# haan6/fm-for-online-recommendation

Measured on AMD Instinct MI355X. Metric: samples/sec online-FM (Criteo-39-field, k=16) FTRL-proximal, higher is better.
Workload: dtype f32

## Files before the change

fm-for-online-recommendation_amd/csrc/fmx_common.h:

```cpp
#pragma once
#include <hip/hip_runtime.h>
#include <hip/hip_ext.h>

#include <cstdarg>
#include <cstdio>
#include <cstdlib>
#include <cstring>
#include <atomic>
#include <mutex>

#include "fmx.h"

#pragma clang fp contract(off)

namespace fmxd {
extern thread_local char g_err[512];
int fail(int code, const char *fmt, ...);
int check_launch(const char *what);

struct Tune {
  int wpb_fwd = 4, wpb_upd = 2;
  int sort_e = 0;
  int inline_fixup = 1;
  int upd_order = 1;
  int online_persistent = 1;
  int afm_online_persistent = 1;
  int afm_pair_online_persistent = 1;
  int sort_ahead = 16;
  int mlp_chain = 1;
  int sort_chunked = 1;
};
Tune &tune();

constexpr int UPD_ORDER_MAX = 128;

constexpr int FMX_COMM_SLOTS = 4;
struct Comm {
  int rank = 0, world = 1, n_blocks = 1;
  bool force = false;
  int block_count[FMX_COMM_MAX_WORLD] = {0}, block_first[FMX_COMM_MAX_WORLD] = {0};
  void *main = nullptr, *pf = nullptr;
  hipStream_t pf_stream = nullptr;
  hipEvent_t fork = nullptr, ready[FMX_COMM_SLOTS] = {nullptr}, free_[FMX_COMM_SLOTS] = {nullptr};
  bool used[FMX_COMM_SLOTS] = {false};
};
int comm_all_gather(Comm *c, int which, const void *send, void *recv, size_t count, hipStream_t st);
int comm_exchange_blocks(Comm *c, const float *send, float *recv, size_t per, hipStream_t st);

constexpr int MLP_BIG_MAX_L = 8;
struct MlpReduceArgs {
  const float *parts[MLP_BIG_MAX_L];
  int out_dim[MLP_BIG_MAX_L], in_dim[MLP_BIG_MAX_L], ldp[MLP_BIG_MAX_L];
  long long grad_off[MLP_BIG_MAX_L];
  float *grads;
  float *params;
  float lr;
  int rule;
  float *m, *v;
  float eps, c1, c2;
  int n_split[MLP_BIG_MAX_L], n_layers;
  const float *loss_b;
  float *loss_out;
  int B;
  float inv_b;
};
int mlp_section_deferred_reduce(const fmx_mlp_t *mlp, int32_t loss_kind, const float *bi, int32_t ld_bi, const float *base, const float *y, int32_t B,
                                float inv_b, void *workspace, float *logit_out, float *dz_out, float *gbi_out, int32_t ld_gbi, float *grads,
                                float lr_apply, float *loss_out, hipStream_t st, MlpReduceArgs *deferred, const char *who = "fmx_mlp_section",
                                float pair_margin = -1.f);
void mlp_launch_reduce(const MlpReduceArgs &a, hipStream_t st);
int mlp_opt_check(const fmx_mlp_t *mlp, int32_t B, const void *workspace, int64_t workspace_bytes, const float *grads, const fmx_mlp_opt_t *opt,
                  int64_t n_steps, const char *who);
int mlp_opt_state_check(const fmx_mlp_opt_t *opt, int64_t n_steps, const char *who);
int mlp_reduce_blocks_per_layer(const MlpReduceArgs &a, int threads);
}
using namespace fmxd;

namespace {

inline bool aligned16(const void *p) { return (reinterpret_cast<uintptr_t>(p) & 15u) == 0; }

constexpr uint32_t SENT = 0xFFFFFFFFu;
constexpr int WAVE = 64;
constexpr int LIST_MAX_G = 16;
constexpr int MAX_SORT_WIDTH = 32768;
constexpr int SORT_CHUNK = 1024;


__device__ __forceinline__ float4 operator+(float4 a, float4 b) { return {a.x + b.x, a.y + b.y, a.z + b.z, a.w + b.w}; }
__device__ __forceinline__ float4 operator-(float4 a, float4 b) { return {a.x - b.x, a.y - b.y, a.z - b.z, a.w - b.w}; }
__device__ __forceinline__ float4 operator*(float4 a, float4 b) { return {a.x * b.x, a.y * b.y, a.z * b.z, a.w * b.w}; }
__device__ __forceinline__ float4 operator*(float a, float4 b) { return {a * b.x, a * b.y, a * b.z, a * b.w}; }
__device__ __forceinline__ float4 splat(float a) { return {a, a, a, a}; }

__device__ __forceinline__ float4 shfl_xor4(float4 v, int m) {
  return {__shfl_xor(v.x, m), __shfl_xor(v.y, m), __shfl_xor(v.z, m), __shfl_xor(v.w, m)};
}
__device__ __forceinline__ float4 shfl_up4(float4 v, int d) {
  return {__shfl_up(v.x, d), __shfl_up(v.y, d), __shfl_up(v.z, d), __shfl_up(v.w, d)};
}
__device__ __forceinline__ float4 shfl4(float4 v, int src) {
  return {__shfl(v.x, src), __shfl(v.y, src), __shfl(v.z, src), __shfl(v.w, src)};
}

__device__ __forceinline__ float rcp_(float x) { return __builtin_amdgcn_rcpf(x); }
__device__ __forceinline__ float sqrt_(float x) { return __builtin_amdgcn_sqrtf(x); }

__device__ __forceinline__ float ftrl_w(float z, float n, const fmx_hyper_t &h) {
  const float denom = fmaf(h.beta + sqrt_(n), h.alpha, h.l2);
  const float w = -(z - copysignf(h.l1, z)) * rcp_(denom);
  return fabsf(z) <= h.l1 ? 0.f : w;
// ... 434 lines not shown
```

fm-for-online-recommendation_amd/csrc/fmx_host.h:

```cpp
#pragma once
#include <type_traits>

#include "fmx_common.h"

namespace fmxd {

struct Workspace {
  uint32_t *sorted;
  size_t sorted_stride;
  uint32_t *runs;
  int32_t *meta;
  int32_t *counter;
  float *parts;
  size_t bytes;
};

struct SortBatch {
  int n_pool = 1, first = 0, n_batches = 1;
  int64_t pool_stride = 0, sorted_stride = 0;
};

int check_table(const fmx_table_t *t);
int check_rule(const fmx_table_t *t, int rule);
int check_adam(const fmx_hyper_t *h, int rule, int64_t n_steps);
int check_sort_geometry(const fmx_table_t *t, int B);
int check_workspace(const fmx_table_t *t, int B, const void *workspace, int64_t workspace_bytes, const char *who);
int check_pair_args(const fmx_table_t *table, const fmx_hyper_t *hyper, const int32_t *idx, int64_t n_pairs, const char *count_name,
                    float margin, const char *who);
int check_list_args(const fmx_table_t *table, const fmx_hyper_t *hyper, const int32_t *idx, int32_t B_lists, int32_t G, int32_t *rows,
                    const char *who);
int named(int rc, const char *who);
int refuse_adaptive(int rule, const char *who);

int forward_impl(const fmx_table_t *table, const fmx_hyper_t *hyper, const int32_t *idx, const float *xv, const float *y,
                 int32_t B, int32_t loss_kind, float inv_b, const fmx_fwd_out_t *out, hipStream_t st);
int sort_impl(const fmx_table_t *table, const int32_t *idx, int32_t B, uint32_t *sorted, uint32_t *runs, int32_t *error,
              hipStream_t st, const SortBatch *mb = nullptr);
bool update_order(const fmx_table_t *table, bool may_fill, uint32_t *order_words);
int update_impl(const fmx_table_t *table, const fmx_hyper_t *hyper, int32_t rule, const Workspace &w,
                const uint32_t *sorted, const float *xv, const float *S, const float *dz_first, const float *dz_bi, const float *gbi,
                int32_t B, const float *loss_b, float inv_b, float *loss_out, hipStream_t st, int32_t *step_counter = nullptr,
                int32_t sample_ld = 0, int32_t *err_flag = nullptr, const MlpReduceArgs *rider = nullptr);
int update_occ_impl(const fmx_table_t *table, const fmx_hyper_t *hyper, int32_t rule, const Workspace &w, const float *xv,
                    const float *dz_first, const float *occ, int32_t ld_occ, int32_t B, const float *loss_b, float inv_b,
                    float *loss_out, hipStream_t st);
int afm_pair_online_buffers(int F, int k, int kp, int t, int attn_rule, bool *moments_in_lds);
int afm_pair_online_launch(const fmx_table_t *table, const fmx_hyper_t *hyper, int32_t rule, const fmx_afm_t *afm, const int32_t *idx,
                           const float *xv, int32_t N_pairs, float margin, float *attn_grad_out, const fmx_mlp_opt_t *opt,
                           float *logit_out, float *loss_out, int32_t *error, int nb, bool moments_in_lds, hipStream_t st);
int list_online_launch(const fmx_table_t *table, const fmx_hyper_t *hyper, int32_t rule, const int32_t *idx, const float *xv, int32_t N,
                       int32_t G, uint8_t *rank_out, float *logit_out, float *loss_out, int32_t *error, hipStream_t st);

}

namespace {

inline int lpr_of(int kp) {
  switch (kp) {
    case 4: return 1;
    case 8: return 2;
    case 16: return 4;
    case 32: return 8;
    case 64: return 16;
    default: return 0;
  }
}

template <class Fn>
decltype(auto) with_lpr(int kp, Fn &&f) {
  switch (lpr_of(kp)) {
    case 1: return f(std::integral_constant<int, 1>{});
    case 2: return f(std::integral_constant<int, 2>{});
    case 4: return f(std::integral_constant<int, 4>{});
    case 8: return f(std::integral_constant<int, 8>{});
    default: return f(std::integral_constant<int, 16>{});
  }
}

template <class Fn>
decltype(auto) with_kp(int kp, Fn &&f) {
  return with_lpr(kp, [&](auto LPR) { return f(std::integral_constant<int, 4 * LPR>{}); });
}

template <int... VS, class Fn>
bool with_one_of(int v, Fn &&f) {
  return ((v == VS && (f(std::integral_constant<int, VS>{}), true)) || ...);
}

template <bool MOMENTS_RULES, class Fn>
bool with_rule_impl(int rule, Fn &&f) {
  using Weights = std::integral_constant<int, FMX_LAYOUT_WEIGHTS>;
  using Moments = std::integral_constant<int, FMX_LAYOUT_MOMENTS>;
  switch (rule) {
    case FMX_RULE_SIGNADAM: f(Weights{}, std::integral_constant<int, FMX_RULE_SIGNADAM>{}); return true;
    case FMX_RULE_SGD: f(Weights{}, std::integral_constant<int, FMX_RULE_SGD>{}); return true;
    case FMX_RULE_FTRL: f(std::integral_constant<int, FMX_LAYOUT_FTRL>{}, std::integral_constant<int, FMX_RULE_FTRL>{}); return true;
    case FMX_RULE_ADAGRAD:
      if constexpr (MOMENTS_RULES) {
        f(Moments{}, std::integral_constant<int, FMX_RULE_ADAGRAD>{});
        return true;
      }
      return false;
    case FMX_RULE_ADAM:
      if constexpr (MOMENTS_RULES) {
        f(Moments{}, std::integral_constant<int, FMX_RULE_ADAM>{});
        return true;
      }
      return false;
    default: return false;
  }
}
template <class Fn>
bool with_rule(int rule, Fn &&f) { return with_rule_impl<true>(rule, f); }
template <class Fn>
bool with_rule_wf(int rule, Fn &&f) { return with_rule_impl<false>(rule, f); }

inline bool adaptive_rule(int rule) { return rule == FMX_RULE_ADAGRAD || rule == FMX_RULE_ADAM; }
inline const char *rule_name(int rule) { return rule == FMX_RULE_ADAM ? "FMX_RULE_ADAM" : "FMX_RULE_ADAGRAD"; }

inline bool mapped(const fmx_table_t *t) { return t->field_cols || t->field_base; }
inline int n_cols(const fmx_table_t *t) { return t->n_cols > 0 ? t->n_cols : t->n_fields; }
// ... 90 lines not shown
```

fm-for-online-recommendation_amd/csrc/fmx_kernels.hip:

```cpp

#include <cmath>

#include "fmx_host.h"

namespace fmxd {

thread_local char g_err[512] = "";

int fail(int code, const char *fmt, ...) {
  va_list ap;
  va_start(ap, fmt);
  vsnprintf(g_err, sizeof(g_err), fmt, ap);
  va_end(ap);
  return code;
}

int check_launch(const char *what) {
  hipError_t e = hipGetLastError();
  if (e != hipSuccess) return fail(FMX_ERR_LAUNCH, "%s: %s", what, hipGetErrorString(e));
  return FMX_OK;
}

}

// ... 444 lines not shown
int check_rule(const fmx_table_t *t, int rule) {
  if (rule == FMX_RULE_FTRL) {
    if (t->layout != FMX_LAYOUT_FTRL) return fail(FMX_ERR_ARG, "FMX_RULE_FTRL needs FMX_LAYOUT_FTRL");
  } else if (rule == FMX_RULE_SIGNADAM || rule == FMX_RULE_SGD) {
    if (t->layout != FMX_LAYOUT_WEIGHTS) return fail(FMX_ERR_ARG, "rule %d needs FMX_LAYOUT_WEIGHTS", rule);
  } else if (adaptive_rule(rule)) {
    if (t->layout != FMX_LAYOUT_MOMENTS) return fail(FMX_ERR_ARG, "%s needs FMX_LAYOUT_MOMENTS", rule_name(rule));
  } else {
    return fail(FMX_ERR_ARG, "unknown rule %d", rule);
  }
  return FMX_OK;
}

int check_adam(const fmx_hyper_t *h, int rule, int64_t n_steps) {
  if (rule != FMX_RULE_ADAM || !h) return FMX_OK;
  if (!(h->beta1 >= 0.f && h->beta1 < 1.f && h->beta2 >= 0.f && h->beta2 < 1.f))
    return fail(FMX_ERR_ARG, "FMX_RULE_ADAM: beta1 = %g and beta2 = %g must lie in [0, 1)", h->beta1, h->beta2);
  if (h->step < 0 || (int64_t)h->step + n_steps > INT32_MAX)
    return fail(FMX_ERR_ARG, "FMX_RULE_ADAM: step = %d must be >= 0 and step + steps of the call <= 2^31 - 1", h->step);
  return FMX_OK;
}

int check_sort_geometry(const fmx_table_t *t, int B) {
  if (B < 1) return fail(FMX_ERR_ARG, "B must be >= 1");
  const int Bp = fmx_sorted_width(B);
  if (Bp > MAX_SORT_WIDTH)
    return fail(FMX_ERR_UNSUPPORTED, "batch %d exceeds the LDS sort width %d", B, MAX_SORT_WIDTH);
  const int bbits = fmx_sorted_bbits(B);
  if ((uint64_t)(max_sort_rows(t) - 1) >= (uint64_t)(SENT >> bbits))
    return fail(FMX_ERR_UNSUPPORTED, "largest sort field (%lld rows) and batch %d do not fit a 32-bit (index, sample) composite: "
                "split the large fields (fmx_table_t.sort_offsets)", (long long)max_sort_rows(t), B);
  return FMX_OK;
}

int check_workspace(const fmx_table_t *t, int B, const void *workspace, int64_t workspace_bytes, const char *who) {
  if (!workspace) return fail(FMX_ERR_ARG, "%s: null workspace", who);
  if (!aligned16(workspace)) return fail(FMX_ERR_ALIGN, "%s: workspace must be 16-byte aligned", who);
  const int64_t need = (int64_t)carve(t, B, nullptr).bytes;
  if (workspace_bytes < need)
    return fail(FMX_ERR_SHAPE, "%s: workspace of %lld bytes, %lld needed for B = %d and %d sort fields (fmx_workspace_bytes)", who,
                (long long)workspace_bytes, (long long)need, B, n_sort_fields(t));
  return FMX_OK;
}

int named(int rc, const char *who) {
  if (rc != FMX_OK && !strstr(g_err, who)) {
    char msg[sizeof(g_err)];
    snprintf(msg, sizeof(msg), "%s", g_err);
    snprintf(g_err, sizeof(g_err), "%s: %s", who, msg);
  }
  return rc;
}

int check_pair_args(const fmx_table_t *table, const fmx_hyper_t *hyper, const int32_t *idx, int64_t n_pairs, const char *count_name,
                    float margin, const char *who) {
  if (!table) return fail(FMX_ERR_ARG, "%s: table is null", who);
  if (int rc = check_table(table)) return named(rc, who);
  if (!hyper) return fail(FMX_ERR_ARG, "%s: hyper is null", who);
  if (!idx) return fail(FMX_ERR_ARG, "%s: idx is null", who);
  if (n_pairs < 1) return fail(FMX_ERR_ARG, "%s: %s = %lld must be >= 1", who, count_name, (long long)n_pairs);
  if (!(margin >= 0.f) || !std::isfinite(margin)) return fail(FMX_ERR_ARG, "%s: margin = %g must be finite and >= 0", who, (double)margin);
  if (mapped(table))
    return fail(FMX_ERR_UNSUPPORTED, "%s: tables whose fields are pieces of index columns (field_cols / field_base) are not taken", who);
  return FMX_OK;
}

int check_list_args(const fmx_table_t *table, const fmx_hyper_t *hyper, const int32_t *idx, int32_t B_lists, int32_t G, int32_t *rows,
                    const char *who) {
  if (int rc = check_pair_args(table, hyper, idx, B_lists, "B_lists", 0.f, who)) return rc;
  if (G < 2) return fail(FMX_ERR_ARG, "%s: G = %d: a list is a positive and at least one negative (G >= 2)", who, G);
  if (G > LIST_MAX_G) return fail(FMX_ERR_UNSUPPORTED, "%s: G = %d: at most %d rows per list (one workgroup holds a list's waves)", who, G, LIST_MAX_G);
  if ((int64_t)B_lists * G > INT32_MAX) return fail(FMX_ERR_ARG, "%s: B_lists = %d, G = %d: B_lists * G rows exceed int32", who, B_lists, G);
  *rows = B_lists * G;
  return FMX_OK;
}

Tune &tune() {
  static Tune t = [] {
    Tune x;
    if (const char *e = getenv("FMX_WPB_FWD")) x.wpb_fwd = atoi(e);
    if (const char *e = getenv("FMX_WPB_UPD")) x.wpb_upd = atoi(e);
    if (const char *e = getenv("FMX_SORT_E")) x.sort_e = atoi(e);
    if (const char *e = getenv("FMX_SORT_AHEAD")) x.sort_ahead = atoi(e);
    if (const char *e = getenv("FMX_ONLINE_PERSISTENT")) x.online_persistent = atoi(e);
    if (const char *e = getenv("FMX_INLINE_FIXUP")) x.inline_fixup = atoi(e);
    if (const char *e = getenv("FMX_SORT_CHUNKED")) x.sort_chunked = atoi(e);
    if (const char *e = getenv("FMX_UPD_ORDER")) x.upd_order = atoi(e);
    if (const char *e = getenv("FMX_MLP_CHAIN")) x.mlp_chain = atoi(e);
    auto ok = [](int v) { return v == 1 || v == 2 || v == 4; };
    if (!ok(x.wpb_fwd)) x.wpb_fwd = 4;
    if (!ok(x.wpb_upd)) x.wpb_upd = 2;
    return x;
  }();
  return t;
}
}
namespace {

struct Side {
  hipStream_t stream = nullptr;
  hipStream_t main = nullptr;
  hipEvent_t fork = nullptr, sorted[2] = {nullptr, nullptr}, consumed[2] = {nullptr, nullptr};
  hipEvent_t user_fork = nullptr, user_join = nullptr;
};

Side *side_for_current_device() {
  static std::mutex mu;
  static Side sides[64];
  int dev = 0;
  if (hipGetDevice(&dev) != hipSuccess || dev < 0 || dev >= 64) return nullptr;
  std::lock_guard<std::mutex> lock(mu);
  Side &sd = sides[dev];
  if (!sd.stream) {
    int lo = 0, hi = 0;
    (void)hipDeviceGetStreamPriorityRange(&lo, &hi);
    if (hipStreamCreateWithPriority(&sd.stream, hipStreamNonBlocking, lo) != hipSuccess) return nullptr;
    if (hipStreamCreateWithPriority(&sd.main, hipStreamNonBlocking, hi) != hipSuccess) return nullptr;
    bool ok = hipEventCreateWithFlags(&sd.fork, hipEventDisableTiming) == hipSuccess &&
              hipEventCreateWithFlags(&sd.user_fork, hipEventDisableTiming) == hipSuccess &&
              hipEventCreateWithFlags(&sd.user_join, hipEventDisableTiming) == hipSuccess;
    for (int i = 0; i < 2 && ok; ++i) {
      ok = hipEventCreateWithFlags(&sd.sorted[i], hipEventDisableTiming) == hipSuccess &&
           hipEventCreateWithFlags(&sd.consumed[i], hipEventDisableTiming) == hipSuccess;
    }
    if (!ok) return nullptr;
  }
  return &sd;
}

struct UpdOrders {
  struct Entry {
    const int64_t *offs = nullptr;
    int F = 0;
    int64_t n_rows = 0, max_rows = 0;
    bool known = false;
    uint8_t order[2][UPD_ORDER_MAX];
  };
  static constexpr int N = 8;
  Entry e[N];
  int next = 0;
};

}
namespace fmxd {

bool update_order(const fmx_table_t *table, bool may_fill, uint32_t *order_words) {
  memset(order_words, 0, UPD_ORDER_MAX);
  const int mode = tune().upd_order, F = n_sort_fields(table);
  if ((mode != 1 && mode != 2) || F < 1 || F > UPD_ORDER_MAX) return false;
  static std::mutex mu;
  static UpdOrders per_device[64];
  int dev = 0;
  if (hipGetDevice(&dev) != hipSuccess || dev < 0 || dev >= 64) return false;
  const int64_t *offs = sort_offsets(table);
  std::lock_guard<std::mutex> lock(mu);
  UpdOrders &c = per_device[dev];
  UpdOrders::Entry *hit = nullptr;
  for (UpdOrders::Entry &x : c.e)
    if (x.offs == offs && x.F == F && x.n_rows == table->n_rows && x.max_rows == max_sort_rows(table)) hit = &x;
  if (!hit) {
    if (!may_fill) return false;
    hit = &c.e[c.next];
    c.next = (c.next + 1) % UpdOrders::N;
    hit->offs = offs;
    hit->F = F;
    hit->n_rows = table->n_rows;
    hit->max_rows = max_sort_rows(table);
    int64_t off[UPD_ORDER_MAX + 1], rows[UPD_ORDER_MAX];
    hipStreamCaptureMode cm = hipStreamCaptureModeRelaxed;
    const bool swapped = hipThreadExchangeStreamCaptureMode(&cm) == hipSuccess;
    hit->known = hipMemcpy(off, offs, sizeof(int64_t) * (size_t)(F + 1), hipMemcpyDeviceToHost) == hipSuccess;
    if (swapped) (void)hipThreadExchangeStreamCaptureMode(&cm);
    if (!hit->known) (void)hipGetLastError();
    for (int f = 0; f < F && hit->known; ++f) rows[f] = off[f + 1] - off[f];
    if (hit->known) hit->known = upd_order_of(rows, F, 1, hit->order[0]) == F && upd_order_of(rows, F, 2, hit->order[1]) == F;
  }
  if (!hit->known) return false;
  memcpy(order_words, hit->order[mode - 1], (size_t)F);
  return true;
}

}
namespace {

constexpr int OVERLAP_MIN_BATCH = 512;

template <int LPR, int NPASS, bool MAPPED = false, bool PAIR = false>
void launch_forward_np(const FwdArgs &a, int layout, hipStream_t st) {
  const int wpb = PAIR && tune().wpb_fwd < 2 ? 2 : tune().wpb_fwd;
  const dim3 grid((a.B + wpb - 1) / wpb), block(64 * wpb);
  if (layout == FMX_LAYOUT_FTRL) hipLaunchKernelGGL((k_fm_forward<LPR, FMX_LAYOUT_FTRL, NPASS, MAPPED, PAIR>), grid, block, 0, st, a);
  else hipLaunchKernelGGL((k_fm_forward<LPR, FMX_LAYOUT_WEIGHTS, NPASS, MAPPED, PAIR>), grid, block, 0, st, a);
}

template <int LPR, bool PAIR = false>
void launch_forward(const FwdArgs &a, int layout, hipStream_t st) {
  const int slots = WAVE / LPR;
  const int np = (a.F + slots - 1) / slots;
  if constexpr (!PAIR) {
    if (a.fcols || a.fbase) {
      launch_forward_np<LPR, 0, true>(a, layout, st);
      return;
    }
  }
  if (!with_one_of<1, 2, 3, 4>(np, [&](auto NP) { launch_forward_np<LPR, NP, false, PAIR>(a, layout, st); }))
    launch_forward_np<LPR, 0, false, PAIR>(a, layout, st);
}

template <int LPR, bool Q = false>
void launch_forward_list(const FwdArgs &a, int layout, hipStream_t st) {
  const int G = a.list_g, wpb = G * (4 / G > 1 ? 4 / G : 1);
  const dim3 grid((a.B + wpb - 1) / wpb), block(64 * wpb);
  const int slots = WAVE / LPR, np = (a.F + slots - 1) / slots;
  auto launch = [&](auto NP) {
    if constexpr (Q) {
      if (layout == FMX_LAYOUT_FTRL) hipLaunchKernelGGL((k_fm_forward_listq<LPR, FMX_LAYOUT_FTRL, NP>), grid, block, 0, st, a);
      else hipLaunchKernelGGL((k_fm_forward_listq<LPR, FMX_LAYOUT_WEIGHTS, NP>), grid, block, 0, st, a);
    } else {
      if (layout == FMX_LAYOUT_FTRL) hipLaunchKernelGGL((k_fm_forward_list<LPR, FMX_LAYOUT_FTRL, NP>), grid, block, 0, st, a);
      else hipLaunchKernelGGL((k_fm_forward_list<LPR, FMX_LAYOUT_WEIGHTS, NP>), grid, block, 0, st, a);
    }
  };
  if (!with_one_of<1, 2, 3, 4>(np, launch)) launch(std::integral_constant<int, 0>{});
}

template <int E>
void launch_sort(SortArgs a, hipStream_t st) {
  const int threads = a.Bp / E;
  uint32_t lds = (uint32_t)(a.Bp * sizeof(uint32_t));
  if (a.Bp <= RADIX_SMALL_WIDTH && threads >= 64) {
    a.small_bits = RADIX_SMALL_BITS;
    const uint32_t need = (uint32_t)radix_small_lds_bytes(a.Bp, threads);
    if (need > lds) lds = need;
  }
  const int grid = a.n_batches >= 8 ? 8 * a.F * ((a.n_batches + 7) / 8) : a.F * a.n_batches;
  hipLaunchKernelGGL((k_sort_occ<E>), dim3(grid), dim3(threads), lds, st, a);
}

int prepare_sort(int B) {
  if ((size_t)fmx_sorted_width(B) * 4 <= 64 * 1024) return FMX_OK;
  static std::mutex mu;
  static bool raised = false;
  std::lock_guard<std::mutex> lock(mu);
  if (!raised) {
    hipError_t e = hipFuncSetAttribute(reinterpret_cast<const void *>(k_sort_occ<8>), hipFuncAttributeMaxDynamicSharedMemorySize, MAX_SORT_WIDTH * 4);
    if (e == hipSuccess) e = hipFuncSetAttribute(reinterpret_cast<const void *>(k_sort_occ<16>), hipFuncAttributeMaxDynamicSharedMemorySize, MAX_SORT_WIDTH * 4);
    if (e == hipSuccess) e = hipFuncSetAttribute(reinterpret_cast<const void *>(k_sort_occ<32>), hipFuncAttributeMaxDynamicSharedMemorySize, MAX_SORT_WIDTH * 4);
    if (e != hipSuccess) return fail(FMX_ERR_LAUNCH, "hipFuncSetAttribute: %s", hipGetErrorString(e));
    raised = true;
  }
  return FMX_OK;
}

int prepare_merge(int Bp) {
  if ((size_t)(Bp + Bp / 32) * 4 <= 64 * 1024) return FMX_OK;
  static std::mutex mu;
  static bool raised = false;
  std::lock_guard<std::mutex> lock(mu);
  if (!raised) {
    hipError_t e = hipFuncSetAttribute(reinterpret_cast<const void *>(k_sort_merge), hipFuncAttributeMaxDynamicSharedMemorySize,
                                       (MAX_SORT_WIDTH + MAX_SORT_WIDTH / 32) * 4);
    if (e != hipSuccess) return fail(FMX_ERR_LAUNCH, "hipFuncSetAttribute: %s", hipGetErrorString(e));
    raised = true;
  }
  return FMX_OK;
}

}

int fmxd::sort_impl(const fmx_table_t *table, const int32_t *idx, int32_t B, uint32_t *sorted, uint32_t *runs, int32_t *error,
                    hipStream_t st, const SortBatch *mb) {
  SortArgs a;
  a.n_pool = mb ? mb->n_pool : 1;
  a.pool_first = mb ? mb->first : 0;
  a.n_batches = mb ? mb->n_batches : 1;
  a.pool_stride = mb ? mb->pool_stride : 0;
  a.sorted_stride = mb ? mb->sorted_stride : 0;
  a.idx = idx;
  a.foff = table->field_offsets;
  a.soff = sort_offsets(table);
  a.cols = sort_cols(table);
  a.sorted = sorted;
  a.error = error;
  a.B = B;
  a.F = n_sort_fields(table);
  a.Fi = n_cols(table);
  a.small_bits = 0;
  a.fcols = table->field_cols;
  a.fbase = table->field_base;
  a.Bp = fmx_sorted_width(B);
  a.bbits = fmx_sorted_bbits(B);
  if (a.Bp >= (tune().sort_chunked > 1 ? 2 * SORT_CHUNK : SORT_CHUNKED_MIN_WIDTH) && tune().sort_chunked && runs &&
      (a.n_batches <= 2 || tune().sort_chunked > 1)) {
    if (int rc = prepare_merge(a.Bp)) return rc;
    ChunkArgs c;
    c.s = a;
    c.runs = runs;
    c.runs_stride = (int64_t)align_up((size_t)a.F * a.Bp * 4, 256) / 4;
    c.C = a.Bp / SORT_CHUNK;
    const int units1 = a.n_batches * c.C, grid1 = 8 * a.F * ((units1 + 7) / 8);
    hipLaunchKernelGGL(k_sort_chunk, dim3(grid1), dim3(SORT_CHUNK_THREADS), 0, st, c);
    const int units2 = a.n_batches * a.F, grid2 = 8 * c.C * ((units2 + 7) / 8);
    hipLaunchKernelGGL(k_sort_merge, dim3(grid2), dim3(SORT_CHUNK_THREADS), (uint32_t)((a.Bp + a.Bp / 32) * sizeof(uint32_t)), st, c);
    return check_launch("k_sort_chunk / k_sort_merge");
  }
  if (int rc = prepare_sort(B)) return rc;
  int E = a.Bp <= 64 ? 1 : a.Bp <= 128 ? 2 : a.Bp <= 4096 ? 4 : a.Bp <= 8192 ? 8 : a.Bp <= 16384 ? 16 : 32;
  const int want = tune().sort_e;
  if (want > E && want <= 32 && (want & (want - 1)) == 0 && a.Bp / want >= 64) E = want;
  if (!with_one_of<1, 2, 4, 8, 16>(E, [&](auto E_) { launch_sort<E_>(a, st); })) launch_sort<32>(a, st);
  return check_launch("k_sort_occ");
}

namespace {

int sort_pool(const fmx_table_t *table, const int32_t *idx_pool, int n_pool, int B, int first_step, int n, const Workspace &w,
              uint32_t *sorted, int32_t *error, hipStream_t st) {
  SortBatch mb;
  mb.n_pool = n_pool;
  mb.first = first_step % n_pool;
  mb.n_batches = n;
  mb.pool_stride = (int64_t)B * (int64_t)n_cols(table);
  mb.sorted_stride = (int64_t)w.sorted_stride;
  return sort_impl(table, idx_pool, B, sorted, w.runs, error, st, &mb);
}

struct Detour {
  Side *sd;
  hipStream_t user, st;
  Detour(Side *side, hipStream_t stream) : sd(stream == nullptr ? side : nullptr), user(stream), st(stream) {
    if (!sd) return;
    (void)hipEventRecord(sd->user_fork, user);
    st = sd->main;
    (void)hipStreamWaitEvent(st, sd->user_fork, 0);
  }
  ~Detour() {
    if (!sd) return;
    (void)hipEventRecord(sd->user_join, st);
    (void)hipStreamWaitEvent(user, sd->user_join, 0);
  }
  Detour(const Detour &) = delete;
  Detour &operator=(const Detour &) = delete;
};

template <class BeforeUpdate, class Update>
int pool_loop(const fmx_table_t *table, const int32_t *idx_pool, const float *y_pool, int n_pool, int B, int n_steps,
              const Workspace &w, int32_t *error, hipStream_t stream, BeforeUpdate &&before_update, Update &&update) {
  Side *sd = (B >= OVERLAP_MIN_BATCH && n_steps > 0) ? side_for_current_device() : nullptr;
  const Detour detour(sd, stream);
  const hipStream_t st = detour.st;
  const size_t F = (size_t)n_cols(table);
  int ahead = tune().sort_ahead;
  if (ahead < 1) ahead = 1;
  if (ahead > SORT_AHEAD_MAX) ahead = SORT_AHEAD_MAX;
  auto group_size = [&](int g, int first_step) {
    int n = g == 0 ? 4 : ahead;
    if (n > ahead) n = ahead;
    if (n > n_steps - first_step) n = n_steps - first_step;
    return n;
  };
  auto sort_group = [&](int g, int first_step, int n, hipStream_t where) -> int {
    return sort_pool(table, idx_pool, n_pool, B, first_step, n, w, w.sorted + (size_t)(g & 1) * ahead * w.sorted_stride, error, where);
  };
  int rc = FMX_OK;
  if (sd) {
    (void)hipEventRecord(sd->fork, st);
    (void)hipStreamWaitEvent(sd->stream, sd->fork, 0);
    rc = sort_group(0, 0, group_size(0, 0), sd->stream);
    (void)hipEventRecord(sd->sorted[0], sd->stream);
  }
  int first_step = 0;
  for (int g = 0; first_step < n_steps && rc == FMX_OK; ++g) {
    const int n = group_size(g, first_step);
    const int next_first = first_step + n;
    if (!sd) rc = sort_group(g, first_step, n, st);
    for (int i = 0; i < n && rc == FMX_OK; ++i) {
      const int s = first_step + i, j = s % n_pool;
      rc = before_update(s, idx_pool + (size_t)j * B * F, y_pool ? y_pool + (size_t)j * B : nullptr, st);
      if (sd && i == 0) (void)hipStreamWaitEvent(st, sd->sorted[g & 1], 0);
      if (rc == FMX_OK) rc = update(s, w.sorted + ((size_t)(g & 1) * ahead + i) * w.sorted_stride, st);
      if (sd && i == 0 && next_first < n_steps && rc == FMX_OK) {
        if (g >= 1) (void)hipStreamWaitEvent(sd->stream, sd->consumed[(g + 1) & 1], 0);
        rc = sort_group(g + 1, next_first, group_size(g + 1, next_first), sd->stream);
        (void)hipEventRecord(sd->sorted[(g + 1) & 1], sd->stream);
      }
    }
    if (sd) (void)hipEventRecord(sd->consumed[g & 1], st);
    first_step = next_first;
  }
  return rc;
}

FwdArgs fill_fwd(const fmx_table_t *table, const fmx_hyper_t *hyper, const int32_t *idx, const float *xv, const float *y,
                 int32_t B, int32_t loss_kind, float inv_b, const fmx_fwd_out_t *out) {
  FwdArgs a;
  a.ldS = out->sample_ld > 0 ? out->sample_ld : table->kp;
  a.ld1 = out->sample_ld > 0 ? out->sample_ld : 1;
  a.rows = table->rows;
  a.foff = table->field_offsets;
  a.bias = table->bias;
  a.idx = idx;
  a.xv = xv;
  a.y = y;
  a.out = *out;
  a.h = kernel_hyper(hyper, -1);
  a.B = B;
  a.F = table->n_fields;
  a.Fc = n_cols(table);
  a.fcols = table->field_cols;
  a.fbase = table->field_base;
  a.kp = table->kp;
  a.stride = table->row_stride;
  a.zoff = table->z_offset;
  a.loss_kind = loss_kind;
  a.inv_b = inv_b;
  a.margin = 0.f;
  return a;
}

}

int fmxd::forward_impl(const fmx_table_t *table, const fmx_hyper_t *hyper, const int32_t *idx, const float *xv, const float *y,
                       int32_t B, int32_t loss_kind, float inv_b, const fmx_fwd_out_t *out, hipStream_t st) {
  const FwdArgs a = fill_fwd(table, hyper, idx, xv, y, B, loss_kind, inv_b, out);
  with_lpr(table->kp, [&](auto LPR) { launch_forward<LPR>(a, table->layout, st); });
  return check_launch("k_fm_forward");
}

namespace {

template <int LPR>
int launch_forward_part(const PartArgs &a, int np, int n_local_blocks, hipStream_t st) {
  const int per_wave = (WAVE / LPR) >> a.sl_log2, waves = (a.B + per_wave - 1) / per_wave;
  const dim3 grid((waves + 3) / 4, n_local_blocks), block(256);
  if (!with_one_of<1, 2, 3, 4>(np, [&](auto NP) { hipLaunchKernelGGL((k_fm_forward_part<LPR, NP>), grid, block, 0, st, a); }))
    return fail(FMX_ERR_UNSUPPORTED, "fmx_fm_forward_partial: more than 4 fields per lane group");
  return check_launch("k_fm_forward_part");
}

template <int LPR, int LAYOUT>
int launch_forward_finish_g(const FinishArgs &a, int G, hipStream_t st) {
  const int waves = (a.B + (WAVE / LPR) - 1) / (WAVE / LPR);
  const dim3 grid((waves + 3) / 4), block(256);
  if (!with_one_of<1, 2, 4, 8, 16>(G, [&](auto G_) { hipLaunchKernelGGL((k_fm_forward_finish<LPR, LAYOUT, G_>), grid, block, 0, st, a); }))
    return fail(FMX_ERR_ARG, "fmx_fm_forward_finish: n_owners must be 1, 2, 4, 8 or 16");
// ... 39 lines not shown
  return with_lpr(table->kp, [&](auto LPR) { return launch_forward_part<LPR>(a, np, n_local_blocks, st); });
}

int check_forward_args(const fmx_table_t *table, const fmx_hyper_t *hyper, const int32_t *idx, const float *y, int32_t B,
                       int32_t loss_kind, const fmx_fwd_out_t *out) {
  if (int rc = check_table(table)) return rc;
  if (!hyper || !idx || !out) return fail(FMX_ERR_ARG, "fmx_fm_forward: null argument");
  if (B < 1) return fail(FMX_ERR_ARG, "B must be >= 1");
  if (loss_kind < FMX_LOSS_NONE || loss_kind > FMX_LOSS_BCE_SIGMOID) return fail(FMX_ERR_ARG, "unknown loss %d", loss_kind);
  if (loss_kind != FMX_LOSS_NONE && !y) return fail(FMX_ERR_ARG, "a loss needs labels y");
  if ((out->S && !aligned16(out->S)) || (out->bi && !aligned16(out->bi)))
    return fail(FMX_ERR_ALIGN, "S and bi must be 16-byte aligned");
  if (out->sample_ld != 0 && (out->sample_ld < table->kp || out->sample_ld % 4))
    return fail(FMX_ERR_SHAPE, "sample_ld=%d must be 0 or a multiple of 4 that is >= kp", out->sample_ld);
  return FMX_OK;
}

int check_step_args(const fmx_table_t *table, const fmx_hyper_t *hyper, int32_t rule, int32_t loss_kind, int32_t B,
                    const void *workspace, const fmx_fwd_out_t *fwd) {
  if (int rc = check_table(table)) return rc;
  if (int rc = check_rule(table, rule)) return rc;
  if (int rc = check_sort_geometry(table, B)) return rc;
  if (!hyper || !workspace) return fail(FMX_ERR_ARG, "null hyper / workspace");
  if (int rc = check_adam(hyper, rule, 1)) return rc;
  if (!aligned16(workspace)) return fail(FMX_ERR_ALIGN, "workspace must be 16-byte aligned");
  if (!fwd || !fwd->S || !fwd->dz || !fwd->loss) return fail(FMX_ERR_ARG, "fwd->S, fwd->loss, fwd->dz are required");
  if (!aligned16(fwd->S) || !aligned16(fwd->dz) || !aligned16(fwd->loss))
    return fail(FMX_ERR_ALIGN, "fwd->S, fwd->dz and fwd->loss must be 16-byte aligned");
  if (loss_kind != FMX_LOSS_BCE_LOGITS && loss_kind != FMX_LOSS_BCE_SIGMOID) return fail(FMX_ERR_ARG, "a step needs a loss");
  return FMX_OK;
}

template <class Forward>
int step_run(const fmx_table_t *table, const fmx_table_t *tu, const fmx_hyper_t *hyper, int32_t rule, const int32_t *idx, const float *xv,
             const float *y, int32_t rows, float inv_b, const Workspace &w, const fmx_fwd_out_t *fwd, float *loss_out, hipStream_t st,
             Forward &&forward) {
  if (int rc = sort_impl(table, idx, rows, w.sorted, w.runs, fwd->error, st)) return rc;
  if (int rc = forward(idx, xv, y, st)) return rc;
  return update_impl(tu, hyper, rule, w, w.sorted, xv, fwd->S, fwd->dz, fwd->dz, nullptr, rows, fwd->loss, inv_b, loss_out, st, nullptr,
                     fwd->sample_ld, fwd->error);
}

template <class Forward>
int stream_run(const fmx_table_t *table, const fmx_table_t *tu, const fmx_hyper_t *hyper, int32_t rule, const int32_t *idx_pool,
               const float *y_pool, int32_t n_pool, int32_t rows, float inv_b, int32_t n_steps, const Workspace &w, const fmx_fwd_out_t *fwd,
               float *loss_out, hipStream_t st, Forward &&forward) {
  auto before_update = [&](int, const int32_t *idx, const float *y, hipStream_t s_) { return forward(idx, nullptr, y, s_); };
  auto update = [&](int s, const uint32_t *sorted, hipStream_t s_) {
    const fmx_hyper_t hs = hyper_at_step(hyper, rule, s);
    return update_impl(tu, &hs, rule, w, sorted, nullptr, fwd->S, fwd->dz, fwd->dz, nullptr, rows, fwd->loss, inv_b,
                       loss_out ? loss_out + s : nullptr, s_, nullptr, fwd->sample_ld, fwd->error);
  };
  return pool_loop(table, idx_pool, y_pool, n_pool, rows, n_steps, w, fwd->error, st, before_update, update);
}

inline auto point_forward(const fmx_table_t *table, const fmx_hyper_t *hyper, int32_t B, int32_t loss_kind, float inv_b,
                          const fmx_fwd_out_t *fwd) {
  return [=](const int32_t *idx, const float *xv, const float *y, hipStream_t st) {
    return forward_impl(table, hyper, idx, xv, y, B, loss_kind, inv_b, fwd, st);
  };
}

int check_pool_steps(int32_t n_pool, int32_t n_steps, const char *who) {
  if (n_pool < 1) return fail(FMX_ERR_ARG, "%s: n_pool = %d must be >= 1", who, n_pool);
  if (n_steps < 0) return fail(FMX_ERR_ARG, "%s: n_steps = %d must be >= 0", who, n_steps);
  return FMX_OK;
}

#include "fmx_pair.inc"
#include "fmx_list.inc"

}

extern "C" {

int fmx_version(void) { return FMX_VERSION; }

int fmx_set_option(const char *name, int value) {
  if (!name) return fail(FMX_ERR_ARG, "fmx_set_option: null name");
  Tune &t = tune();
  int *slot = nullptr;
  if (!strcmp(name, "inline_fixup")) slot = &t.inline_fixup;
  else if (!strcmp(name, "sort_ahead")) slot = &t.sort_ahead;
  else if (!strcmp(name, "online_persistent")) slot = &t.online_persistent;
  else if (!strcmp(name, "afm_online_persistent")) slot = &t.afm_online_persistent;
  else if (!strcmp(name, "afm_pair_online_persistent")) slot = &t.afm_pair_online_persistent;
  else if (!strcmp(name, "sort_chunked")) slot = &t.sort_chunked;
  else if (!strcmp(name, "upd_order")) slot = &t.upd_order;
  else if (!strcmp(name, "mlp_chain")) slot = &t.mlp_chain;
  else return fail(FMX_ERR_ARG, "fmx_set_option: unknown option '%s'", name);
  const int old = *slot;
  *slot = value;
  return old;
}

const char *fmx_last_error_string(void) { return g_err; }

int fmx_update_order(const int64_t *rows, int32_t n, int32_t mode, uint8_t *order) {
  if (!rows || !order) return fail(FMX_ERR_ARG, "fmx_update_order: null argument");
  if (n < 1) return fail(FMX_ERR_ARG, "fmx_update_order: n = %d must be >= 1", (int)n);
  if (mode < 0 || mode > 2) return fail(FMX_ERR_ARG, "fmx_update_order: mode = %d is none of 0, 1, 2", (int)mode);
  return upd_order_of(rows, n, mode, order);
}

int fmx_sorted_width(int B) {
  int w = 64;
  while (w < B && w < (1 << 30)) w <<= 1;
  return w;
}

int fmx_sorted_bbits(int B) {
  int w = fmx_sorted_width(B), bits = 0;
  while ((1 << bits) < w) ++bits;
  return bits;
}

int64_t fmx_workspace_bytes(const fmx_table_t *table, int32_t B) {
  if (check_table(table) != FMX_OK) return FMX_ERR_ARG;
  if (B < 1) return fail(FMX_ERR_ARG, "B must be >= 1");
  return (int64_t)carve(table, B, nullptr).bytes;
}

int fmx_fm_forward(const fmx_table_t *table, const fmx_hyper_t *hyper, const int32_t *idx, const float *xv,
                   const float *y, int32_t B, int32_t loss_kind, float inv_b, const fmx_fwd_out_t *out,
                   fmx_stream_t stream) {
  if (int rc = check_forward_args(table, hyper, idx, y, B, loss_kind, out)) return rc;
  return forward_impl(table, hyper, idx, xv, y, B, loss_kind, inv_b, out, static_cast<hipStream_t>(stream));
}

int fmx_fm_forward_partial(const fmx_table_t *table, const int32_t *idx, const float *xv, int32_t B, int32_t n_blocks,
                           int32_t n_local_blocks, int32_t group, float *parts_out, int32_t *error, fmx_stream_t stream) {
  if (int rc = check_table(table)) return rc;
  if (!idx || !parts_out) return fail(FMX_ERR_ARG, "fmx_fm_forward_partial: null argument");
  if (B < 1) return fail(FMX_ERR_ARG, "B must be >= 1");
  if (!aligned16(parts_out)) return fail(FMX_ERR_ALIGN, "parts_out must be 16-byte aligned");
  return part_impl(table, idx, xv, B, n_blocks, n_local_blocks, group, parts_out, error, static_cast<hipStream_t>(stream));
}

int fmx_fm_forward_finish(const fmx_hyper_t *hyper, const float *bias, int32_t layout, int32_t kp, const float *parts,
                          int64_t owner_stride, int32_t n_owners, const float *y, int32_t B, int32_t loss_kind, float inv_b,
                          const fmx_fwd_out_t *out, fmx_stream_t stream) {
  if (!hyper || !bias || !parts || !out) return fail(FMX_ERR_ARG, "fmx_fm_forward_finish: null argument");
  if (layout != FMX_LAYOUT_WEIGHTS && layout != FMX_LAYOUT_FTRL && layout != FMX_LAYOUT_MOMENTS)
    return fail(FMX_ERR_ARG, "unknown layout %d", layout);
  if (!lpr_of(kp)) return fail(FMX_ERR_SHAPE, "kp=%d must be 4/8/16/32/64", kp);
  if (B < 1) return fail(FMX_ERR_ARG, "B must be >= 1");
  if (loss_kind < FMX_LOSS_NONE || loss_kind > FMX_LOSS_BCE_SIGMOID) return fail(FMX_ERR_ARG, "unknown loss %d", loss_kind);
  if (loss_kind != FMX_LOSS_NONE && !y) return fail(FMX_ERR_ARG, "a loss needs labels y");
  if (!aligned16(parts) || owner_stride % 4 || (out->S && !aligned16(out->S)) || (out->bi && !aligned16(out->bi)))
    return fail(FMX_ERR_ALIGN, "parts, S and bi must be 16-byte aligned, owner_stride a multiple of 4");
  if (out->sample_ld != 0 && (out->sample_ld < kp || out->sample_ld % 4))
    return fail(FMX_ERR_SHAPE, "sample_ld=%d must be 0 or a multiple of 4 that is >= kp", out->sample_ld);
  FinishArgs a;
  a.parts = parts;
  a.rank_stride = owner_stride;
  a.bias = bias;
  a.y = y;
  a.out = *out;
  a.h = kernel_hyper(hyper, -1);
  a.B = B;
  a.loss_kind = loss_kind;
  a.ldS = out->sample_ld > 0 ? out->sample_ld : kp;
  a.ld1 = out->sample_ld > 0 ? out->sample_ld : 1;
  a.inv_b = inv_b;
  hipStream_t st = static_cast<hipStream_t>(stream);
  return with_lpr(kp, [&](auto LPR) { return launch_forward_finish<LPR>(a, layout, n_owners, st); });
}

int fmx_sort_occurrences(const fmx_table_t *table, const int32_t *idx, int32_t B, void *workspace, int64_t workspace_bytes, int32_t *error,
                         fmx_stream_t stream) {
  if (int rc = check_table(table)) return rc;
  if (!idx || !workspace) return fail(FMX_ERR_ARG, "fmx_sort_occurrences: null argument");
  if (!aligned16(workspace)) return fail(FMX_ERR_ALIGN, "workspace must be 16-byte aligned");
  if (int rc = check_sort_geometry(table, B)) return rc;
  if (int rc = check_workspace(table, B, workspace, workspace_bytes, "fmx_sort_occurrences")) return rc;
// ... 401 lines not shown
```

fm-for-online-recommendation_amd/csrc/fmx_sort.inc:

```

struct SortArgs {
  int32_t n_pool, pool_first, n_batches;
  int64_t pool_stride, sorted_stride;
  const int32_t *idx;
  const int64_t *foff;
  const int64_t *soff;
  const int32_t *cols;
  const int32_t *fcols;
  const int32_t *fbase;
  uint32_t *sorted;
  int32_t *error;
  int32_t B, F, Bp, bbits;
  int32_t Fi;
  int32_t small_bits;
};

template <int E, int LJ>
__device__ __forceinline__ void bitonic_lane_stage(uint32_t (&v)[E], int i0, int lane, int k) {
  const bool lower = (lane & LJ) == 0;
  const bool up = (i0 & k) == 0;
  const bool take_min = lower == up;
#pragma unroll
  for (int r = 0; r < E; ++r) {
    const uint32_t o = xor_lane<LJ>(v[r], lane);
// ... 171 lines not shown
  if (bad && a.error) *a.error = 1;
  uint32_t *st = bits <= RADIX_D ? st_out : nullptr;
  const int n_pass = (bits + RADIX_D - 1) / RADIX_D;
  int shift = a.bbits, left = bits;
  uint32_t *src = keys, *dst = alt;
  for (int ps = 0; ps < n_pass; ++ps) {
    const int d = (left + (n_pass - ps) - 1) / (n_pass - ps);
    const bool last = ps + 1 == n_pass;
    radix_pass(src, last ? nullptr : dst, out, cnt, lrank, sc, Bp, shift, d, pad_from, last ? st : nullptr);
    shift += d;
    left -= d;
    uint32_t *t = src;
    src = dst;
    dst = t;
  }
}

template <int E>
__device__ __forceinline__ void sort_field(const SortArgs &a, int f, uint32_t *sm) {
  const int tid = threadIdx.x, nt = blockDim.x;
  if (a.small_bits > 0) {
    const uint32_t piece_rows = (uint32_t)(a.soff[f + 1] - a.soff[f]);
    const int bits = piece_rows ? 32 - __clz((int)piece_rows) : 1;
    if (bits <= a.small_bits) {
      radix_field<true>(a, f, a.idx, a.sorted + (size_t)f * a.Bp, sm, nullptr);
      return;
    }
  }
  uint32_t v[E];
  load_composites<E>(a, f, tid * E, v);
  const int wave_span = 64 * E;
  uint32_t *dst = a.sorted + (size_t)f * a.Bp;
  const int half = a.Bp >> 1;
  for (int k = 2; k <= a.Bp; k <<= 1) {
    int j = k >> 1;
    if (j >= wave_span) {
#pragma unroll
      for (int r = 0; r < E; ++r) sm[tid * E + r] = v[r];
      __syncthreads();
      for (; j >= wave_span; j >>= 1) {
        for (int t = tid; t < half; t += nt) {
          const int i = 2 * t - (t & (j - 1));
          const int l = i + j;
          const uint32_t x = sm[i], y = sm[l];
          const bool up = (i & k) == 0;
          if ((x > y) == up) { sm[i] = y; sm[l] = x; }
        }
        __syncthreads();
      }
#pragma unroll
      for (int r = 0; r < E; ++r) v[r] = sm[tid * E + r];
      __syncthreads();
    }
    bitonic_local<E>(v, tid, k, j);
  }
#pragma unroll
  for (int r = 0; r < E; ++r) dst[(size_t)tid * E + r] = v[r];
}

__device__ __forceinline__ bool xcd_unit(int n_units, int n_inner, int &unit, int &inner) {
  const int b = blockIdx.x, x = b & 7, s = b >> 3;
  inner = s % n_inner;
  unit = (s / n_inner) * 8 + x;
  return unit < n_units;
}

template <int E>
__global__ __launch_bounds__(1024) void k_sort_occ(SortArgs a) {
  extern __shared__ uint32_t sm[];
  int j, f;
  if (a.n_batches >= 8) {
    if (!xcd_unit(a.n_batches, a.F, j, f)) return;
  } else {
    j = blockIdx.x / a.F;
    f = blockIdx.x - j * a.F;
  }
  if (j > 0 || a.pool_stride != 0) {
    a.idx += (size_t)((a.pool_first + j) % a.n_pool) * a.pool_stride;
    a.sorted += (size_t)j * a.sorted_stride;
  }
  sort_field<E>(a, f, sm);
}

constexpr int SORT_CHUNK_E = 4, SORT_CHUNK_THREADS = SORT_CHUNK / SORT_CHUNK_E;
constexpr int SORT_CHUNKED_MIN_WIDTH = 8192;

struct ChunkArgs {
  SortArgs s;
  uint32_t *runs;
  int64_t runs_stride;
  int32_t C;
};

__global__ __launch_bounds__(SORT_CHUNK_THREADS) void k_sort_chunk(ChunkArgs a) {
  constexpr int E = SORT_CHUNK_E;
  __shared__ uint32_t sm[SORT_CHUNK];
  int unit, f;
  if (!xcd_unit(a.s.n_batches * a.C, a.s.F, unit, f)) return;
  const int j = unit / a.C, c = unit - j * a.C;
  const int32_t *idx = a.s.idx + (size_t)((a.s.pool_first + j) % a.s.n_pool) * a.s.pool_stride;
  uint32_t *dst = a.runs + (size_t)j * a.runs_stride + (size_t)f * a.s.Bp + (size_t)c * SORT_CHUNK;
  const int tid = threadIdx.x;
  uint32_t v[E];
  {
    SortArgs sa = a.s;
    sa.idx = idx;
    load_composites<E>(sa, f, c * SORT_CHUNK + tid * E, v);
  }
  constexpr int wave_span = 64 * E;
  for (int k = 2; k <= SORT_CHUNK; k <<= 1) {
    int jj = k >> 1;
    if (jj >= wave_span) {
#pragma unroll
      for (int r = 0; r < E; ++r) sm[tid * E + r] = v[r];
      __syncthreads();
      for (; jj >= wave_span; jj >>= 1) {
        for (int t = tid; t < SORT_CHUNK / 2; t += SORT_CHUNK_THREADS) {
          const int i = 2 * t - (t & (jj - 1));
          const int l = i + jj;
          const uint32_t x = sm[i], y = sm[l];
          const bool up = (i & k) == 0;
          if ((x > y) == up) { sm[i] = y; sm[l] = x; }
        }
        __syncthreads();
      }
#pragma unroll
      for (int r = 0; r < E; ++r) v[r] = sm[tid * E + r];
      __syncthreads();
    }
    bitonic_local<E>(v, tid, k, jj);
  }
  *reinterpret_cast<uint4 *>(dst + tid * E) = uint4{v[0], v[1], v[2], v[3]};
}

__global__ __launch_bounds__(SORT_CHUNK_THREADS) void k_sort_merge(ChunkArgs a) {
  constexpr int E = SORT_CHUNK_E;
  extern __shared__ __attribute__((aligned(16))) uint32_t smem[];
  int unit, c;
  if (!xcd_unit(a.s.n_batches * a.s.F, a.C, unit, c)) return;
  const int j = unit / a.s.F, f = unit - j * a.s.F;
  const uint32_t *src = a.runs + (size_t)j * a.runs_stride + (size_t)f * a.s.Bp;
  uint32_t *dst = a.s.sorted + (size_t)j * a.s.sorted_stride + (size_t)f * a.s.Bp;
  const int tid = threadIdx.x;
  auto at = [](int i) { return i + (i >> 5); };
  {
    uint4 t[8];
    const int n_it = a.s.Bp / (SORT_CHUNK_THREADS * 4);
    for (int it0 = 0; it0 < n_it; it0 += 8) {
#pragma unroll
      for (int u = 0; u < 8; ++u)
        if (it0 + u < n_it) t[u] = *reinterpret_cast<const uint4 *>(src + (it0 + u) * SORT_CHUNK_THREADS * 4 + tid * 4);
#pragma unroll
      for (int u = 0; u < 8; ++u)
        if (it0 + u < n_it) {
          const int i = (it0 + u) * SORT_CHUNK_THREADS * 4 + tid * 4;
          uint32_t *d4 = smem + at(i);
          d4[0] = t[u].x; d4[1] = t[u].y; d4[2] = t[u].z; d4[3] = t[u].w;
        }
    }
  }
  __syncthreads();
  uint32_t v[E];
  int pos[E];
#pragma unroll
  for (int r = 0; r < E; ++r) {
    v[r] = smem[at(c * SORT_CHUNK + tid * E + r)];
// ... 47 lines not shown
```

Baseline: 203.5 million.

## Add CU-resident persistent sort kernel capped to half the CUs for overlapped sorting

Adds a persistent k_sort_occ_resident kernel that loops over (batch, field) units with a grid capped at half the CU count. It pads LDS so only one workgroup fits per CU, and it walks fields in a cached update order. It is used for sort-ahead groups after the first two, so the background sort leaves CUs free for the concurrent update/forward kernels. The trade-off is less sort parallelism, plus extra device-attribute queries on each launch.

```diff
diff --git a/fm-for-online-recommendation_amd/csrc/fmx_common.h b/fm-for-online-recommendation_amd/csrc/fmx_common.h
--- a/fm-for-online-recommendation_amd/csrc/fmx_common.h
+++ b/fm-for-online-recommendation_amd/csrc/fmx_common.h
@@ -27,6 +27,7 @@
   int afm_online_persistent = 1;
   int afm_pair_online_persistent = 1;
   int sort_ahead = 16;
+  int sort_resident = -1;
   int mlp_chain = 1;
   int sort_chunked = 1;
 };
diff --git a/fm-for-online-recommendation_amd/csrc/fmx_host.h b/fm-for-online-recommendation_amd/csrc/fmx_host.h
--- a/fm-for-online-recommendation_amd/csrc/fmx_host.h
+++ b/fm-for-online-recommendation_amd/csrc/fmx_host.h
@@ -18,6 +18,7 @@
 struct SortBatch {
   int n_pool = 1, first = 0, n_batches = 1;
   int64_t pool_stride = 0, sorted_stride = 0;
+  int resident = 0;
 };
 
 int check_table(const fmx_table_t *t);
@@ -37,6 +38,7 @@
 int sort_impl(const fmx_table_t *table, const int32_t *idx, int32_t B, uint32_t *sorted, uint32_t *runs, int32_t *error,
               hipStream_t st, const SortBatch *mb = nullptr);
 bool update_order(const fmx_table_t *table, bool may_fill, uint32_t *order_words);
+bool sort_walk_order(const fmx_table_t *table, uint32_t *order_words);
 int update_impl(const fmx_table_t *table, const fmx_hyper_t *hyper, int32_t rule, const Workspace &w,
                 const uint32_t *sorted, const float *xv, const float *S, const float *dz_first, const float *dz_bi, const float *gbi,
                 int32_t B, const float *loss_b, float inv_b, float *loss_out, hipStream_t st, int32_t *step_counter = nullptr,
diff --git a/fm-for-online-recommendation_amd/csrc/fmx_kernels.hip b/fm-for-online-recommendation_amd/csrc/fmx_kernels.hip
--- a/fm-for-online-recommendation_amd/csrc/fmx_kernels.hip
+++ b/fm-for-online-recommendation_amd/csrc/fmx_kernels.hip
@@ -550,6 +550,7 @@
     if (const char *e = getenv("FMX_WPB_UPD")) x.wpb_upd = atoi(e);
     if (const char *e = getenv("FMX_SORT_E")) x.sort_e = atoi(e);
     if (const char *e = getenv("FMX_SORT_AHEAD")) x.sort_ahead = atoi(e);
+    if (const char *e = getenv("FMX_SORT_RESIDENT")) x.sort_resident = atoi(e);
     if (const char *e = getenv("FMX_ONLINE_PERSISTENT")) x.online_persistent = atoi(e);
     if (const char *e = getenv("FMX_INLINE_FIXUP")) x.inline_fixup = atoi(e);
     if (const char *e = getenv("FMX_SORT_CHUNKED")) x.sort_chunked = atoi(e);
@@ -612,9 +613,9 @@
 }
 namespace fmxd {
 
-bool update_order(const fmx_table_t *table, bool may_fill, uint32_t *order_words) {
+static bool cached_order(const fmx_table_t *table, int mode, bool may_fill, uint32_t *order_words) {
   memset(order_words, 0, UPD_ORDER_MAX);
-  const int mode = tune().upd_order, F = n_sort_fields(table);
+  const int F = n_sort_fields(table);
   if ((mode != 1 && mode != 2) || F < 1 || F > UPD_ORDER_MAX) return false;
   static std::mutex mu;
   static UpdOrders per_device[64];
@@ -648,6 +649,12 @@
   return true;
 }
 
+bool update_order(const fmx_table_t *table, bool may_fill, uint32_t *order_words) {
+  return cached_order(table, tune().upd_order, may_fill, order_words);
+}
+
+bool sort_walk_order(const fmx_table_t *table, uint32_t *order_words) { return cached_order(table, 2, false, order_words); }
+
 }
 namespace {
 
@@ -693,16 +700,59 @@
 }
 
 template <int E>
-void launch_sort(SortArgs a, hipStream_t st) {
-  const int threads = a.Bp / E;
+uint32_t sort_occ_shape(SortArgs &a, int &threads) {
+  threads = a.Bp / E;
   uint32_t lds = (uint32_t)(a.Bp * sizeof(uint32_t));
   if (a.Bp <= RADIX_SMALL_WIDTH && threads >= 64) {
     a.small_bits = RADIX_SMALL_BITS;
     const uint32_t need = (uint32_t)radix_small_lds_bytes(a.Bp, threads);
     if (need > lds) lds = need;
   }
+  return lds;
+}
+
+template <int E>
+void launch_sort(SortArgs a, hipStream_t st) {
+  int threads;
+  const uint32_t lds = sort_occ_shape<E>(a, threads);
   const int grid = a.n_batches >= 8 ? 8 * a.F * ((a.n_batches + 7) / 8) : a.F * a.n_batches;
   hipLaunchKernelGGL((k_sort_occ<E>), dim3(grid), dim3(threads), lds, st, a);
+}
+
+template <int E>
+int launch_sort_resident(SortArgs a, int cap, const fmx_table_t *table, hipStream_t st, bool *launched) {
+  *launched = false;
+  int dev = 0, lds_cu = 0, lds_wg = 0;
+  if (hipGetDevice(&dev) != hipSuccess || hipDeviceGetAttribute(&lds_cu, hipDeviceAttributeMaxSharedMemoryPerMultiprocessor, dev) != hipSuccess ||
+      hipDeviceGetAttribute(&lds_wg, hipDeviceAttributeMaxSharedMemoryPerBlock, dev) != hipSuccess) {
+    (void)hipGetLastError();
+    return FMX_OK;
+  }
+  int threads;
+  uint32_t lds = sort_occ_shape<E>(a, threads);
+  const uint32_t one_per_cu = (uint32_t)align_up((size_t)lds_cu / 2 + 1, 256);
+  if (one_per_cu > lds) lds = one_per_cu;
+  if (lds > (uint32_t)lds_wg) return FMX_OK;
+  if (int rc = raise_lds_limit<k_sort_occ_resident<E>>(lds_wg, "k_sort_occ_resident")) return rc;
+  ResidentSortArgs ra;
+  ra.s = a;
+  const int units = a.n_batches * a.F;
+  ra.n_wg = ((units < cap ? units : cap) + 7) / 8 * 8;
+  ra.ordered = sort_walk_order(table, ra.order) ? 1 : 0;
+  hipLaunchKernelGGL((k_sort_occ_resident<E>), dim3(ra.n_wg), dim3(threads), lds, st, ra);
+  *launched = true;
+  return FMX_OK;
+}
+
+int sort_resident_cap() {
+  const int v = tune().sort_resident;
+  if (v >= 0) return v;
+  int dev = 0, cus = 0;
+  if (hipGetDevice(&dev) != hipSuccess || hipDeviceGetAttribute(&cus, hipDeviceAttributeMultiprocessorCount, dev) != hipSuccess) {
+    (void)hipGetLastError();
+    return 0;
+  }
+  return cus / 2;
 }
 
 int prepare_sort(int B) {
@@ -776,6 +826,13 @@
   int E = a.Bp <= 64 ? 1 : a.Bp <= 128 ? 2 : a.Bp <= 4096 ? 4 : a.Bp <= 8192 ? 8 : a.Bp <= 16384 ? 16 : 32;
   const int want = tune().sort_e;
   if (want > E && want <= 32 && (want & (want - 1)) == 0 && a.Bp / want >= 64) E = want;
+  if (mb && mb->resident > 0 && E <= 16) {
+    bool launched = false;
+    int rc = FMX_OK;
+    with_one_of<1, 2, 4, 8, 16>(E, [&](auto E_) { rc = launch_sort_resident<E_>(a, mb->resident, table, st, &launched); });
+    if (rc != FMX_OK) return rc;
+    if (launched) return check_launch("k_sort_occ_resident");
+  }
   if (!with_one_of<1, 2, 4, 8, 16>(E, [&](auto E_) { launch_sort<E_>(a, st); })) launch_sort<32>(a, st);
   return check_launch("k_sort_occ");
 }
@@ -783,13 +840,14 @@
 namespace {
 
 int sort_pool(const fmx_table_t *table, const int32_t *idx_pool, int n_pool, int B, int first_step, int n, const Workspace &w,
-              uint32_t *sorted, int32_t *error, hipStream_t st) {
+              uint32_t *sorted, int32_t *error, hipStream_t st, int resident = 0) {
   SortBatch mb;
   mb.n_pool = n_pool;
   mb.first = first_step % n_pool;
   mb.n_batches = n;
   mb.pool_stride = (int64_t)B * (int64_t)n_cols(table);
   mb.sorted_stride = (int64_t)w.sorted_stride;
+  mb.resident = resident;
   return sort_impl(table, idx_pool, B, sorted, w.runs, error, st, &mb);
 }
 
@@ -827,8 +885,10 @@
     if (n > n_steps - first_step) n = n_steps - first_step;
     return n;
   };
+  const int resident = sd ? sort_resident_cap() : 0;
   auto sort_group = [&](int g, int first_step, int n, hipStream_t where) -> int {
-    return sort_pool(table, idx_pool, n_pool, B, first_step, n, w, w.sorted + (size_t)(g & 1) * ahead * w.sorted_stride, error, where);
+    return sort_pool(table, idx_pool, n_pool, B, first_step, n, w, w.sorted + (size_t)(g & 1) * ahead * w.sorted_stride, error, where,
+                     sd && g >= 2 ? resident : 0);
   };
   int rc = FMX_OK;
   if (sd) {
@@ -1034,6 +1094,7 @@
   int *slot = nullptr;
   if (!strcmp(name, "inline_fixup")) slot = &t.inline_fixup;
   else if (!strcmp(name, "sort_ahead")) slot = &t.sort_ahead;
+  else if (!strcmp(name, "sort_resident")) slot = &t.sort_resident;
   else if (!strcmp(name, "online_persistent")) slot = &t.online_persistent;
   else if (!strcmp(name, "afm_online_persistent")) slot = &t.afm_online_persistent;
   else if (!strcmp(name, "afm_pair_online_persistent")) slot = &t.afm_pair_online_persistent;
@@ -1042,7 +1103,7 @@
   else if (!strcmp(name, "mlp_chain")) slot = &t.mlp_chain;
   else return fail(FMX_ERR_ARG, "fmx_set_option: unknown option '%s'", name);
   const int old = *slot;
-  *slot = value;
+  *slot = slot == &t.sort_resident && value < 0 ? -1 : value;
   return old;
 }
 
diff --git a/fm-for-online-recommendation_amd/csrc/fmx_sort.inc b/fm-for-online-recommendation_amd/csrc/fmx_sort.inc
--- a/fm-for-online-recommendation_amd/csrc/fmx_sort.inc
+++ b/fm-for-online-recommendation_amd/csrc/fmx_sort.inc
@@ -277,6 +277,36 @@
   sort_field<E>(a, f, sm);
 }
 
+struct ResidentSortArgs {
+  SortArgs s;
+  int32_t n_wg;
+  int32_t ordered;
+  uint32_t order[UPD_ORDER_MAX / 4];
+};
+
+template <int E>
+__global__ __launch_bounds__(1024) void k_sort_occ_resident(ResidentSortArgs ra) {
+  extern __shared__ uint32_t sm[];
+  const SortArgs &a = ra.s;
+  const int x = blockIdx.x & 7, s = blockIdx.x >> 3, per_xcd = ra.n_wg >> 3;
+  const int nb = x < a.n_batches ? (a.n_batches - x + 7) >> 3 : 0;
+  for (int u = s; u < nb * a.F; u += per_xcd) {
+    const int pos = u / nb, j = x + 8 * (u - pos * nb);
+    int f = pos;
+    if (ra.ordered) {
+      typedef const __attribute__((address_space(4))) uint32_t karg_u32;
+      karg_u32 *ka = (karg_u32 *)__builtin_amdgcn_kernarg_segment_ptr();
+      f = (int)((ka[offsetof(ResidentSortArgs, order) / 4 + (pos >> 2)] >> ((pos & 3) * 8)) & 0xFFu);
+      if (f >= a.F) f = pos;
+    }
+    SortArgs ua = a;
+    ua.idx += (size_t)((a.pool_first + j) % a.n_pool) * a.pool_stride;
+    ua.sorted += (size_t)j * a.sorted_stride;
+    sort_field<E>(ua, f, sm);
+    __syncthreads();
+  }
+}
+
 constexpr int SORT_CHUNK_E = 4, SORT_CHUNK_THREADS = SORT_CHUNK / SORT_CHUNK_E;
 constexpr int SORT_CHUNKED_MIN_WIDTH = 8192;
 
```

Result: faster. 208.0 million, median of 6 (+2.2%).
